# gchq/annchor

Hardware: AMD Instinct MI355X
Metric: knn_graph_builds_per_s (1 / Annchor.fit() wall-clock; BASELINE: k-NN graph build time + recall@k) (higher is better)
Workload: dtype int32 bit-vectors (Levenshtein) + f64 (bounds/regression/selection); 1 GPU; load_strings Levenshtein N=1600 n_anchors=15 k=25 p_work=0.12 niters=2; parallelism=one GPU

## Files before the change

### annchor_amd/csrc/model.hip

```cpp
#include "common.h"

#define OLS_T 256
#define ERR_CAP 8192

int ann_dev_flags(annchor_ctx *c)
{
    ANN_TRY(ann_reserve(c, c->dev_flags, sizeof(int32_t) * 16));
    if (!c->dev_flags_clean) {
        ANN_CHECK_HIP(c, hipMemsetAsync(c->dev_flags.p, 0, sizeof(int32_t) * 16, c->stream));
        c->dev_flags_clean = true;
    }
    return ANNCHOR_OK;
}

__device__ __forceinline__ double block_sum(double v, double *sh )
{
#pragma unroll
    for (int off = 32; off > 0; off >>= 1) v += __shfl_xor(v, off);
    __syncthreads();
    if ((threadIdx.x & 63) == 0) sh[threadIdx.x >> 6] = v;
    __syncthreads();
    double s = sh[0];
    for (int w = 1; w < OLS_T / 64; ++w) s += sh[w];
    return s;
}

#define OLS_RCOND 1e-13
struct ModelEdges { double e[MAXBINS + 1]; };
__global__ __launch_bounds__(OLS_T) void k_ols_bins(const double *__restrict__ sfeat, const double *__restrict__ sy, int64_t m,
                                                   DeviceModel *__restrict__ dm, double *__restrict__ scratch, int64_t cap,
                                                   int32_t *__restrict__ flags, ModelEdges ed, int nb)
{
    __shared__ double sh[OLS_T / 64];
    __shared__ int wcnt[OLS_T / 64];
    __shared__ int base_sh;
    const int b = blockIdx.x, tid = threadIdx.x, lane = tid & 63, wave = tid >> 6;
    const double lo = ed.e[b], hi = ed.e[b + 1];
    if (tid == 0) dm->status[b] = 0;
    if (b == 0) {
        if (tid >= nb && tid < MAXBINS) { dm->status[tid] = 0; dm->rows[tid] = 0; }
        if (tid <= nb) dm->reg.e[tid] = ed.e[tid];
        if (tid == 0) { dm->reg.nb = nb; dm->err_status = 0; }
    }
    double *A = scratch + (size_t)b * 4 * cap;
    double *col[4] = {A, A + cap, A + 2 * cap, A + 3 * cap};
    if (tid == 0) base_sh = 0;
    __syncthreads();
    for (int64_t t0 = 0; t0 < m; t0 += OLS_T) {
        const int64_t t = t0 + tid;
        const double d = t < m ? sfeat[4 * t + 2] : 0.0;
        const bool in = t < m && d > lo && d <= hi;
        const unsigned long long bal = __ballot(in);
        if (lane == 0) wcnt[wave] = __popcll(bal);
        __syncthreads();
        int off = base_sh;
        for (int w = 0; w < wave; ++w) off += wcnt[w];
        if (in) {
            const int r = off + __popcll(bal & ((1ull << lane) - 1ull));
            col[0][r] = sfeat[4 * t]; col[1][r] = sfeat[4 * t + 1]; col[2][r] = d; col[3][r] = sy[t];
        }
        __syncthreads();
        if (tid == 0) base_sh += wcnt[0] + wcnt[1] + wcnt[2] + wcnt[3];
        __syncthreads();
    }
    const int n = base_sh;
    if (tid == 0) dm->rows[b] = n;
    if (n < 3) {
        if (tid == 0) {
            dm->status[b] = 2; dm->reg.w[b][0] = dm->reg.w[b][1] = dm->reg.w[b][2] = 0.0; dm->reg.c[b] = 0.0;
            atomicMax(&flags[1], 2);
        }
        return;
    }
    double mean[4];
    for (int k = 0; k < 4; ++k) {
        double s = 0.0;
        for (int r = tid; r < n; r += OLS_T) s += col[k][r];
        mean[k] = block_sum(s, sh) / (double)n;
    }
    for (int k = 0; k < 4; ++k)
        for (int r = tid; r < n; r += OLS_T) col[k][r] -= mean[k];
    __syncthreads();
    double Rd[3], R01 = 0, R02 = 0, R12 = 0, qy[3];
    double cmax = 0.0;
    for (int j = 0; j < 3; ++j) {
        double s = 0.0;
        for (int r = j + tid; r < n; r += OLS_T) s += col[j][r] * col[j][r];
        const double sigma = block_sum(s, sh);
        const double ajj = col[j][j];
        const double alpha = ajj > 0.0 ? -sqrt(sigma) : sqrt(sigma);
        Rd[j] = alpha;
        cmax = fmax(cmax, fabs(alpha));
        const double vtv = 2.0 * (sigma - alpha * ajj);
        __syncthreads();
        if (tid == 0) col[j][j] = ajj - alpha;
        __syncthreads();
        for (int k = j + 1; k < 4; ++k) {
            double dsum = 0.0;
            for (int r = j + tid; r < n; r += OLS_T) dsum += col[j][r] * col[k][r];
            const double dot = block_sum(dsum, sh);
            const double tau = vtv > 0.0 ? 2.0 * dot / vtv : 0.0;
            for (int r = j + tid; r < n; r += OLS_T) col[k][r] -= tau * col[j][r];
            __syncthreads();
        }
        if (j == 0) { R01 = col[1][0]; R02 = col[2][0]; }
        if (j == 1) R12 = col[2][1];
        qy[j] = col[3][j];
    }
    if (tid == 0) {
        const double tol = 1e-10 * cmax;
        int st = 0;
        for (int j = 0; j < 3; ++j)
            if (!(fabs(Rd[j]) > tol)) st = 1;
        double w2 = 0, w1 = 0, w0 = 0;
        if (!st) {
            w2 = qy[2] / Rd[2];
            w1 = (qy[1] - R12 * w2) / Rd[1];
            w0 = ((qy[0] - R01 * w1) - R02 * w2) / Rd[0];
        } else {
            double M[3][3] = {{Rd[0], R01, R02}, {0.0, Rd[1], R12}, {0.0, 0.0, Rd[2]}};
            double V[3][3] = {{1, 0, 0}, {0, 1, 0}, {0, 0, 1}};
            bool conv = false;
            for (int sweep = 0; sweep < 40 && !conv; ++sweep) {
                conv = true;
                for (int p = 0; p < 2; ++p)
                    for (int q = p + 1; q < 3; ++q) {
                        double al = 0, be = 0, ga = 0;
                        for (int r = 0; r < 3; ++r) { al += M[r][p] * M[r][p]; be += M[r][q] * M[r][q]; ga += M[r][p] * M[r][q]; }
                        if (ga == 0.0 || al <= 1e-40 * be || be <= 1e-40 * al || fabs(ga) <= 4.5e-16 * sqrt(al * be)) continue;
                        conv = false;
                        const double zeta = (be - al) / (2.0 * ga);
                        const double tt = (zeta >= 0.0 ? 1.0 : -1.0) / (fabs(zeta) + sqrt(1.0 + zeta * zeta));
                        const double cs = 1.0 / sqrt(1.0 + tt * tt), sn = cs * tt;
                        for (int r = 0; r < 3; ++r) {
                            const double mp = M[r][p], mq = M[r][q];
                            M[r][p] = cs * mp - sn * mq; M[r][q] = sn * mp + cs * mq;
                            const double vp = V[r][p], vq = V[r][q];
                            V[r][p] = cs * vp - sn * vq; V[r][q] = sn * vp + cs * vq;
                        }
                    }
            }
            double sg2[3], smax2 = 0.0;
            for (int i = 0; i < 3; ++i) {
                sg2[i] = (M[0][i] * M[0][i] + M[1][i] * M[1][i]) + M[2][i] * M[2][i];
                smax2 = fmax(smax2, sg2[i]);
            }
            if (conv && smax2 > 0.0) {
                double w[3] = {0, 0, 0};
                for (int i = 0; i < 3; ++i)
                    if (sg2[i] > (OLS_RCOND * OLS_RCOND) * smax2) {
                        const double coef = ((M[0][i] * qy[0] + M[1][i] * qy[1]) + M[2][i] * qy[2]) / sg2[i];
                        for (int r = 0; r < 3; ++r) w[r] += coef * V[r][i];
                    }
                w0 = w[0]; w1 = w[1]; w2 = w[2];
                st = 0;
            } else if (smax2 == 0.0) st = 0;
        }
        dm->status[b] = st;
        if (st) atomicMax(&flags[1], st);
        dm->reg.w[b][0] = w0; dm->reg.w[b][1] = w1; dm->reg.w[b][2] = w2;
        dm->reg.c[b] = mean[3] - ((mean[0] * w0 + mean[1] * w1) + mean[2] * w2);
    }
}

extern "C" int annchor_fit_regression_device(annchor_ctx *c, const double *bins, int32_t nb, int32_t first_iteration, int32_t is_metric)
{
    if (!c || !bins) return ANNCHOR_EINVAL;
    ANN_REQUIRE(c, c->have_features, ANNCHOR_EINVAL, "features not computed");
    ANN_REQUIRE(c, nb >= 1 && nb <= MAXBINS, ANNCHOR_ELIMIT, "1..%d partitions supported", MAXBINS);
    ANN_REQUIRE(c, first_iteration || c->have_RA, ANNCHOR_EINVAL, "RefineApprox not initialised");
    ANN_REQUIRE(c, c->nsamp > 0 && c->sfeat.p && c->sy.p, ANNCHOR_ESTATE, "no device-resident sample (annchor_sample_pairs_device)");
    ANN_REQUIRE(c, c->sfeat_rows == c->nsamp, ANNCHOR_ESTATE,
                "the current sample of %lld pairs has no device-resident feature rows (%lld rows from an earlier annchor_sample_pairs_device)",
                (long long)c->nsamp, (long long)c->sfeat_rows);
    ANN_CHECK_HIP(c, hipSetDevice(c->device));
    const int64_t m = c->nsamp;
    ANN_TRY(ann_reserve(c, c->model, sizeof(DeviceModel)));
    ANN_TRY(ann_reserve(c, c->ols_scratch, sizeof(double) * 4 * (size_t)m * (size_t)nb));
    ANN_TRY(ann_dev_flags(c));
    DeviceModel *dm = c->model.as<DeviceModel>();
    ModelEdges ed;
    for (int k = 0; k <= MAXBINS; ++k) ed.e[k] = k <= nb ? bins[k] : 0.0;
    static_assert(MAXBINS + 1 <= OLS_T, "one thread per edge");
    {
        ProfScope ps(c, "ols_partitions", (double)m * 40.0 * nb);
        k_ols_bins<<<nb, OLS_T, 0, c->stream>>>(c->sfeat.as<double>(), c->sy.as<double>(), m, dm, c->ols_scratch.as<double>(), m,
                                                c->dev_flags.as<int32_t>(), ed, nb);
    }
    ANN_CHECK_HIP(c, hipGetLastError());
    c->model_fitted = true; c->model_nb = nb; c->errs_on_device = false; c->model_cache_valid = false;
    return ann_predict_merge_device(c, &dm->reg, first_iteration, is_metric);
}

__device__ __forceinline__ unsigned long long err_key(double v) { return ann_key_asc(v); }

__global__ __launch_bounds__(1024) void k_err_sort(const double *__restrict__ sfeat, const double *__restrict__ sy,
                                                   const double *__restrict__ spred, int64_t m, DeviceModel *__restrict__ dm,
                                                   double *__restrict__ errs, int nb, int32_t *__restrict__ flags,
                                                   int64_t *__restrict__ errptr_out)
{
    extern __shared__ unsigned long long keys[];
    __shared__ int wcnt[16];
    __shared__ int base_sh;
    __shared__ int pcnt[MAXBINS];
    const int b = blockIdx.x, tid = threadIdx.x, lane = tid & 63, wave = tid >> 6;
    const double lo = dm->reg.e[b], hi = dm->reg.e[b + 1];
    if (tid < MAXBINS) pcnt[tid] = 0;
    __syncthreads();
    for (int64_t t = tid; t < m; t += 1024) {
        const double d = sfeat[4 * t + 2];
        for (int q = 0; q < nb; ++q)
            if (d >= dm->reg.e[q] && d <= dm->reg.e[q + 1]) atomicAdd(&pcnt[q], 1);
    }
    __syncthreads();
    const int n = pcnt[b];
    if (tid == 0) dm->rows[b] = n;
    int64_t my_at = 0;
    for (int q = 0; q < b; ++q) my_at += pcnt[q];
    if (b == 0 && tid == 0) {
        int64_t at = 0;
        int st = 0;
        for (int q = 0; q < nb; ++q) {
            dm->errptr[q] = at;
            errptr_out[q] = at;
            const int64_t r = pcnt[q];
            if (r == 0) st = max(st, 1);
            if (r > ERR_CAP) st = max(st, 2);
            at += r;
        }
        dm->errptr[nb] = at;
        errptr_out[nb] = at;
        dm->err_status = st;
        if (st) flags[2] = st;
    }
    if (n == 0 || n > ERR_CAP) return;
    int P2 = 1;
    while (P2 < n) P2 <<= 1;
    for (int t = tid; t < P2; t += 1024) keys[t] = ~0ull;
    if (tid == 0) base_sh = 0;
    __syncthreads();
    for (int64_t t0 = 0; t0 < m; t0 += 1024) {
        const int64_t t = t0 + tid;
        const double d = t < m ? sfeat[4 * t + 2] : 0.0;
        const bool in = t < m && d >= lo && d <= hi;
        const unsigned long long bal = __ballot(in);
        if (lane == 0) wcnt[wave] = __popcll(bal);
        __syncthreads();
        int off = base_sh;
        for (int w = 0; w < wave; ++w) off += wcnt[w];
        if (in) keys[off + __popcll(bal & ((1ull << lane) - 1ull))] = err_key(sy[t] - spred[t]);
        __syncthreads();
        if (tid == 0) {
            int s = 0;
            for (int w = 0; w < 16; ++w) s += wcnt[w];
            base_sh += s;
        }
        __syncthreads();
    }
    for (int k = 2; k <= P2; k <<= 1)
        for (int j = k >> 1; j > 0; j >>= 1) {
            for (int t = tid; t < P2; t += 1024) {
                const int p = t ^ j;
                if (p > t) {
                    const unsigned long long a = keys[t], bb = keys[p];
                    const bool up = (t & k) == 0;
                    if ((a > bb) == up) { keys[t] = bb; keys[p] = a; }
                }
            }
            __syncthreads();
        }
    double *out = errs + my_at;
    for (int t = tid; t < n; t += 1024) out[t] = ann_key_asc_inv(keys[t]);
}

extern "C" int annchor_fit_errors_device(annchor_ctx *c)
{
    if (!c) return ANNCHOR_EINVAL;
    ANN_REQUIRE(c, c->model_fitted && c->nsamp > 0 && c->spred.p, ANNCHOR_ESTATE, "annchor_fit_regression_device first");
    ANN_REQUIRE(c, c->sfeat_rows == c->nsamp, ANNCHOR_ESTATE, "the sample changed since annchor_fit_regression_device");
    ANN_CHECK_HIP(c, hipSetDevice(c->device));
    const int nb = c->model_nb;
    const int64_t m = c->nsamp;
    DeviceModel *dm = c->model.as<DeviceModel>();
    ANN_TRY(ann_reserve(c, c->errs, sizeof(double) * 2 * (size_t)m));
    ANN_TRY(ann_reserve(c, c->errptr, sizeof(int64_t) * (size_t)(MAXBINS + 1)));
    {
        ProfScope ps(c, "error_residual_lists", (double)m * 32.0 * nb);
        const size_t lds = sizeof(unsigned long long) * ERR_CAP;
        ANN_CHECK_HIP(c, hipFuncSetAttribute((const void *)k_err_sort, hipFuncAttributeMaxDynamicSharedMemorySize, (int)lds));
        k_err_sort<<<nb, 1024, lds, c->stream>>>(c->sfeat.as<double>(), c->sy.as<double>(), c->spred.as<double>(), m, dm, c->errs.as<double>(),
                                                 nb, c->dev_flags.as<int32_t>(), c->errptr.as<int64_t>());
    }
    ANN_CHECK_HIP(c, hipGetLastError());
    c->errs_on_device = true; c->model_cache_valid = false;
    return ANNCHOR_OK;
}

extern "C" int annchor_model_download(annchor_ctx *c, double *W, double *cc, int32_t *status, int64_t *err_ptr, int32_t *flags)
{
    if (!c || !W || !cc || !status || !flags) return ANNCHOR_EINVAL;
    ANN_REQUIRE(c, c->model.p && c->model_nb > 0, ANNCHOR_ESTATE, "no model on this context");
    ANN_CHECK_HIP(c, hipSetDevice(c->device));
    DeviceModel h;
    int32_t f[16];
    ANN_TRY(ann_dev_flags(c));
    ANN_TRY(ann_d2h2(c, &h, c->model.p, sizeof h, f, c->dev_flags.p, sizeof f));
    for (int b = 0; b < c->model_nb; ++b) {
        W[3 * b] = h.reg.w[b][0]; W[3 * b + 1] = h.reg.w[b][1]; W[3 * b + 2] = h.reg.w[b][2];
        cc[b] = h.reg.c[b];
        status[b] = h.status[b];
    }
    if (err_ptr)
        for (int b = 0; b <= c->model_nb; ++b) err_ptr[b] = h.errptr[b];
    flags[0] = f[0]; flags[1] = f[1]; flags[2] = f[2];
    if (f[0] | f[1] | f[2]) {
        ANN_CHECK_HIP(c, hipMemsetAsync(c->dev_flags.p, 0, sizeof(int32_t) * 16, c->stream));
    }
    return ANNCHOR_OK;
}

int ann_model_prefetch_begin(annchor_ctx *c, unsigned char *at, size_t room, size_t *used)
{
    *used = 0;
    c->model_cache_valid = false;
    if (!(c->model_fitted && c->errs_on_device && c->model.p && c->errs.p && c->model_nb > 0)) return ANNCHOR_OK;
    const size_t eb = sizeof(double) * 2 * (size_t)c->nsamp;
    const size_t off_f = (sizeof(DeviceModel) + 63) & ~(size_t)63, off_e = off_f + 64;
    if (off_e + eb > room) return ANNCHOR_OK;
    ANN_TRY(ann_dev_flags(c));
    ANN_CHECK_HIP(c, hipMemcpyAsync(at, c->model.p, sizeof(DeviceModel), hipMemcpyDeviceToHost, c->stream));
    ANN_CHECK_HIP(c, hipMemcpyAsync(at + off_f, c->dev_flags.p, sizeof(int32_t) * 16, hipMemcpyDeviceToHost, c->stream));
    if (eb) ANN_CHECK_HIP(c, hipMemcpyAsync(at + off_e, c->errs.p, eb, hipMemcpyDeviceToHost, c->stream));
    c->model_cache_errs = eb;
    *used = off_e + eb;
    return ANNCHOR_OK;
}
void ann_model_prefetch_end(annchor_ctx *c, const unsigned char *at, size_t used)
{
    if (!used) return;
    c->model_cache.assign(at, at + used);
    c->model_cache_valid = true;
}

extern "C" int annchor_model_download_with_errors(annchor_ctx *c, double *W, double *cc, int32_t *status, int64_t *err_ptr, int32_t *flags,
                                                  double *errs, int64_t errs_cap, int64_t *n_errs)
{
    if (!c || !W || !cc || !status || !flags || !err_ptr || !errs || !n_errs) return ANNCHOR_EINVAL;
    ANN_REQUIRE(c, c->model.p && c->model_nb > 0, ANNCHOR_ESTATE, "no model on this context");
    ANN_REQUIRE(c, c->errs_on_device && c->errs.p, ANNCHOR_ESTATE, "no device-resident residual lists");
    ANN_CHECK_HIP(c, hipSetDevice(c->device));
    size_t eb = sizeof(double) * (size_t)std::min<int64_t>(errs_cap, 2 * c->nsamp);
    const size_t off_f = (sizeof(DeviceModel) + 63) & ~(size_t)63, off_e = off_f + 64;
    const bool cached = c->model_cache_valid && c->model_cache.size() >= off_e + c->model_cache_errs;
    c->model_cache_valid = false;
    if (!cached && (!c->pin || off_e + eb > annchor_ctx::PIN_DL_BYTES)) {
        ANN_TRY(annchor_model_download(c, W, cc, status, err_ptr, flags));
        *n_errs = err_ptr[c->model_nb];
        ANN_REQUIRE(c, *n_errs <= errs_cap, ANNCHOR_EINVAL, "residual lists hold %lld entries, room for %lld", (long long)*n_errs, (long long)errs_cap);
        return annchor_errors_download(c, errs, *n_errs);
    }
    ANN_TRY(ann_dev_flags(c));
    const unsigned char *slot = c->pin + (size_t)annchor_ctx::PIN_SLOTS * annchor_ctx::PIN_SLOT_BYTES;
    if (cached) {
        slot = c->model_cache.data();
        eb = c->model_cache_errs;
    } else {
        unsigned char *dst = c->pin + (size_t)annchor_ctx::PIN_SLOTS * annchor_ctx::PIN_SLOT_BYTES;
        ANN_CHECK_HIP(c, hipMemcpyAsync(dst, c->model.p, sizeof(DeviceModel), hipMemcpyDeviceToHost, c->stream));
        ANN_CHECK_HIP(c, hipMemcpyAsync(dst + off_f, c->dev_flags.p, sizeof(int32_t) * 16, hipMemcpyDeviceToHost, c->stream));
        if (eb) ANN_CHECK_HIP(c, hipMemcpyAsync(dst + off_e, c->errs.p, eb, hipMemcpyDeviceToHost, c->stream));
        ANN_CHECK_HIP(c, ann_sync(c, __func__));
    }
    const DeviceModel &h = *reinterpret_cast<const DeviceModel *>(slot);
    const int32_t *f = reinterpret_cast<const int32_t *>(slot + off_f);
    for (int b = 0; b < c->model_nb; ++b) {
        W[3 * b] = h.reg.w[b][0]; W[3 * b + 1] = h.reg.w[b][1]; W[3 * b + 2] = h.reg.w[b][2];
        cc[b] = h.reg.c[b];
        status[b] = h.status[b];
    }
    for (int b = 0; b <= c->model_nb; ++b) err_ptr[b] = h.errptr[b];
    flags[0] = f[0]; flags[1] = f[1]; flags[2] = f[2];
    *n_errs = err_ptr[c->model_nb];
    if (*n_errs < 0 || (size_t)*n_errs * sizeof(double) > eb || *n_errs > errs_cap) *n_errs = -1;
    else memcpy(errs, slot + off_e, sizeof(double) * (size_t)*n_errs);
    if (f[0] | f[1] | f[2]) ANN_CHECK_HIP(c, hipMemsetAsync(c->dev_flags.p, 0, sizeof(int32_t) * 16, c->stream));
    return ANNCHOR_OK;
}

extern "C" int annchor_errors_download(annchor_ctx *c, double *errs, int64_t n_errs)
{
    if (!c || (n_errs > 0 && !errs)) return ANNCHOR_EINVAL;
    ANN_REQUIRE(c, c->errs_on_device && c->errs.p, ANNCHOR_ESTATE, "no device-resident residual lists");
    if (n_errs == 0) return ANNCHOR_OK;
    ANN_CHECK_HIP(c, hipSetDevice(c->device));
    return ann_d2h(c, errs, c->errs.p, sizeof(double) * (size_t)n_errs);
}
```

Before: 369.1 graphs/s.

## Restructure OLS and error-sort kernels with LDS staging, fused reductions, register bitonic sort

```diff
diff --git a/annchor_amd/csrc/model.hip b/annchor_amd/csrc/model.hip
--- a/annchor_amd/csrc/model.hip
+++ b/annchor_amd/csrc/model.hip
@@ -1,7 +1,14 @@
 #include "common.h"
+#include <atomic>
 
 #define OLS_T 256
+#define OLS_PER 8
+#define OLS_TRIP (OLS_T * OLS_PER)
+#define OLS_LDS_ROWS 4096
 #define ERR_CAP 8192
+#define ERR_T 1024
+#define ERR_PER 8
+#define ERR_TRIP (ERR_T * ERR_PER)
 
 int ann_dev_flags(annchor_ctx *c)
 {
@@ -13,27 +20,108 @@
     return ANNCHOR_OK;
 }
 
-__device__ __forceinline__ double block_sum(double v, double *sh )
-{
-#pragma unroll
-    for (int off = 32; off > 0; off >>= 1) v += __shfl_xor(v, off);
+static int ann_lds_once(annchor_ctx *c, const void *fn, int which, size_t bytes)
+{
+    static std::atomic<bool> done[2][64];
+    const int d = c->device;
+    const bool memo = d >= 0 && d < 64;
+    if (memo && done[which][d].load(std::memory_order_acquire)) return ANNCHOR_OK;
+    ANN_CHECK_HIP(c, hipFuncSetAttribute(fn, hipFuncAttributeMaxDynamicSharedMemorySize, (int)bytes));
+    if (memo) done[which][d].store(true, std::memory_order_release);
+    return ANNCHOR_OK;
+}
+
+template <int NV> __device__ __forceinline__ void block_sums(double (&v)[NV], double (*sh)[4][OLS_T / 64], int &par)
+{
+#pragma unroll
+    for (int k = 0; k < NV; ++k) {
+#pragma unroll
+        for (int off = 32; off > 0; off >>= 1) v[k] += __shfl_xor(v[k], off);
+    }
+    if ((threadIdx.x & 63) == 0) {
+#pragma unroll
+        for (int k = 0; k < NV; ++k) sh[par][k][threadIdx.x >> 6] = v[k];
+    }
     __syncthreads();
-    if ((threadIdx.x & 63) == 0) sh[threadIdx.x >> 6] = v;
-    __syncthreads();
-    double s = sh[0];
-    for (int w = 1; w < OLS_T / 64; ++w) s += sh[w];
-    return s;
+#pragma unroll
+    for (int k = 0; k < NV; ++k) {
+        double s = sh[par][k][0];
+#pragma unroll
+        for (int w = 1; w < OLS_T / 64; ++w) s += sh[par][k][w];
+        v[k] = s;
+    }
+    par ^= 1;
 }
 
 #define OLS_RCOND 1e-13
 struct ModelEdges { double e[MAXBINS + 1]; };
+struct OlsFactor { double mean[4], Rd[3], R01, R02, R12, qy[3], cmax; };
+
+__device__ __forceinline__ void ols_factor(double *A, const size_t cap, const int n, double (*sh)[4][OLS_T / 64], int &par, OlsFactor &f)
+{
+    const int tid = threadIdx.x;
+    double *col[4] = {A, A + cap, A + 2 * cap, A + 3 * cap};
+    double s4[4] = {0.0, 0.0, 0.0, 0.0};
+    for (int r = tid; r < n; r += OLS_T) {
+#pragma unroll
+        for (int k = 0; k < 4; ++k) s4[k] += col[k][r];
+    }
+    block_sums<4>(s4, sh, par);
+#pragma unroll
+    for (int k = 0; k < 4; ++k) f.mean[k] = s4[k] / (double)n;
+    double sg[1] = {0.0};
+    for (int r = tid; r < n; r += OLS_T) {
+        const double x0 = col[0][r] - f.mean[0];
+        col[0][r] = x0;
+        sg[0] += x0 * x0;
+#pragma unroll
+        for (int k = 1; k < 4; ++k) col[k][r] -= f.mean[k];
+    }
+    f.R01 = f.R02 = f.R12 = 0.0;
+    f.cmax = 0.0;
+#pragma unroll
+    for (int j = 0; j < 3; ++j) {
+        if (j > 0) {
+            sg[0] = 0.0;
+            for (int r = j + tid; r < n; r += OLS_T) sg[0] += col[j][r] * col[j][r];
+        }
+        block_sums<1>(sg, sh, par);
+        const double sigma = sg[0];
+        const double ajj = col[j][j];
+        const double alpha = ajj > 0.0 ? -sqrt(sigma) : sqrt(sigma);
+        f.Rd[j] = alpha;
+        f.cmax = fmax(f.cmax, fabs(alpha));
+        const double vtv = 2.0 * (sigma - alpha * ajj);
+        const double v0 = ajj - alpha;
+        double dot[3] = {0.0, 0.0, 0.0};
+        for (int r = j + tid; r < n; r += OLS_T) {
+            const double vj = r == j ? v0 : col[j][r];
+#pragma unroll
+            for (int k = j + 1; k < 4; ++k) dot[k - 1] += vj * col[k][r];
+        }
+        block_sums<3>(dot, sh, par);
+        double tau[3];
+#pragma unroll
+        for (int k = j + 1; k < 4; ++k) tau[k - 1] = vtv > 0.0 ? 2.0 * dot[k - 1] / vtv : 0.0;
+        for (int r = j + tid; r < n; r += OLS_T) {
+            const double vj = r == j ? v0 : col[j][r];
+#pragma unroll
+            for (int k = j + 1; k < 4; ++k) col[k][r] -= tau[k - 1] * vj;
+        }
+        __syncthreads();
+        if (j == 0) { f.R01 = col[1][0]; f.R02 = col[2][0]; }
+        if (j == 1) f.R12 = col[2][1];
+        f.qy[j] = col[3][j];
+    }
+}
+
 __global__ __launch_bounds__(OLS_T) void k_ols_bins(const double *__restrict__ sfeat, const double *__restrict__ sy, int64_t m,
                                                    DeviceModel *__restrict__ dm, double *__restrict__ scratch, int64_t cap,
-                                                   int32_t *__restrict__ flags, ModelEdges ed, int nb)
-{
-    __shared__ double sh[OLS_T / 64];
-    __shared__ int wcnt[OLS_T / 64];
-    __shared__ int base_sh;
+                                                   int32_t *__restrict__ flags, ModelEdges ed, int nb, int lrows)
+{
+    extern __shared__ double ols_lds[];
+    __shared__ double sh[2][4][OLS_T / 64];
+    __shared__ int wcnt[2][OLS_PER][OLS_T / 64];
     const int b = blockIdx.x, tid = threadIdx.x, lane = tid & 63, wave = tid >> 6;
     const double lo = ed.e[b], hi = ed.e[b + 1];
     if (tid == 0) dm->status[b] = 0;
@@ -42,28 +130,48 @@
         if (tid <= nb) dm->reg.e[tid] = ed.e[tid];
         if (tid == 0) { dm->reg.nb = nb; dm->err_status = 0; }
     }
-    double *A = scratch + (size_t)b * 4 * cap;
-    double *col[4] = {A, A + cap, A + 2 * cap, A + 3 * cap};
-    if (tid == 0) base_sh = 0;
-    __syncthreads();
-    for (int64_t t0 = 0; t0 < m; t0 += OLS_T) {
-        const int64_t t = t0 + tid;
-        const double d = t < m ? sfeat[4 * t + 2] : 0.0;
-        const bool in = t < m && d > lo && d <= hi;
-        const unsigned long long bal = __ballot(in);
-        if (lane == 0) wcnt[wave] = __popcll(bal);
+    double *G = scratch + (size_t)b * 4 * cap;
+    const double2 *__restrict__ sf2 = reinterpret_cast<const double2 *>(sfeat);
+    const unsigned long long below = (1ull << lane) - 1ull;
+    int base = 0, wp = 0;
+    for (int64_t t0 = 0; t0 < m; t0 += OLS_TRIP) {
+        double2 fa[OLS_PER], fb[OLS_PER];
+        double yv[OLS_PER];
+        unsigned long long bal[OLS_PER];
+#pragma unroll
+        for (int i = 0; i < OLS_PER; ++i) {
+            const int64_t t = t0 + i * OLS_T + tid, tc = t < m ? t : m - 1;
+            fa[i] = sf2[2 * tc]; fb[i] = sf2[2 * tc + 1]; yv[i] = sy[tc];
+        }
+#pragma unroll
+        for (int i = 0; i < OLS_PER; ++i) {
+            const int64_t t = t0 + i * OLS_T + tid;
+            bal[i] = __ballot(t < m && fb[i].x > lo && fb[i].x <= hi);
+            if (lane == 0) wcnt[wp][i][wave] = __popcll(bal[i]);
+        }
         __syncthreads();
-        int off = base_sh;
-        for (int w = 0; w < wave; ++w) off += wcnt[w];
-        if (in) {
-            const int r = off + __popcll(bal & ((1ull << lane) - 1ull));
-            col[0][r] = sfeat[4 * t]; col[1][r] = sfeat[4 * t + 1]; col[2][r] = d; col[3][r] = sy[t];
-        }
-        __syncthreads();
-        if (tid == 0) base_sh += wcnt[0] + wcnt[1] + wcnt[2] + wcnt[3];
-        __syncthreads();
-    }
-    const int n = base_sh;
+        int run = base;
+#pragma unroll
+        for (int i = 0; i < OLS_PER; ++i) {
+            int off = 0;
+#pragma unroll
+            for (int w = 0; w < OLS_T / 64; ++w) {
+                if (w == wave) off = run;
+                run += wcnt[wp][i][w];
+            }
+            if ((bal[i] >> lane) & 1ull) {
+                const int r = off + __popcll(bal[i] & below);
+                if (r < lrows) {
+                    ols_lds[r] = fa[i].x; ols_lds[lrows + r] = fa[i].y; ols_lds[2 * lrows + r] = fb[i].x; ols_lds[3 * lrows + r] = yv[i];
+                } else {
+                    G[r] = fa[i].x; G[cap + r] = fa[i].y; G[2 * cap + r] = fb[i].x; G[3 * cap + r] = yv[i];
+                }
+            }
+        }
+        base = run;
+        wp ^= 1;
+    }
+    const int n = base;
     if (tid == 0) dm->rows[b] = n;
     if (n < 3) {
         if (tid == 0) {
@@ -72,41 +180,20 @@
         }
         return;
     }
-    double mean[4];
-    for (int k = 0; k < 4; ++k) {
-        double s = 0.0;
-        for (int r = tid; r < n; r += OLS_T) s += col[k][r];
-        mean[k] = block_sum(s, sh) / (double)n;
-    }
-    for (int k = 0; k < 4; ++k)
-        for (int r = tid; r < n; r += OLS_T) col[k][r] -= mean[k];
     __syncthreads();
-    double Rd[3], R01 = 0, R02 = 0, R12 = 0, qy[3];
-    double cmax = 0.0;
-    for (int j = 0; j < 3; ++j) {
-        double s = 0.0;
-        for (int r = j + tid; r < n; r += OLS_T) s += col[j][r] * col[j][r];
-        const double sigma = block_sum(s, sh);
-        const double ajj = col[j][j];
-        const double alpha = ajj > 0.0 ? -sqrt(sigma) : sqrt(sigma);
-        Rd[j] = alpha;
-        cmax = fmax(cmax, fabs(alpha));
-        const double vtv = 2.0 * (sigma - alpha * ajj);
+    OlsFactor f;
+    int par = 0;
+    if (n <= lrows) ols_factor(ols_lds, (size_t)lrows, n, sh, par, f);
+    else {
+        for (int r = tid; r < lrows; r += OLS_T) {
+#pragma unroll
+            for (int k = 0; k < 4; ++k) G[(size_t)k * cap + r] = ols_lds[k * lrows + r];
+        }
         __syncthreads();
-        if (tid == 0) col[j][j] = ajj - alpha;
-        __syncthreads();
-        for (int k = j + 1; k < 4; ++k) {
-            double dsum = 0.0;
-            for (int r = j + tid; r < n; r += OLS_T) dsum += col[j][r] * col[k][r];
-            const double dot = block_sum(dsum, sh);
-            const double tau = vtv > 0.0 ? 2.0 * dot / vtv : 0.0;
-            for (int r = j + tid; r < n; r += OLS_T) col[k][r] -= tau * col[j][r];
-            __syncthreads();
-        }
-        if (j == 0) { R01 = col[1][0]; R02 = col[2][0]; }
-        if (j == 1) R12 = col[2][1];
-        qy[j] = col[3][j];
-    }
+        ols_factor(G, (size_t)cap, n, sh, par, f);
+    }
+    const double *mean = f.mean, *Rd = f.Rd, *qy = f.qy;
+    const double R01 = f.R01, R02 = f.R02, R12 = f.R12, cmax = f.cmax;
     if (tid == 0) {
         const double tol = 1e-10 * cmax;
         int st = 0;
@@ -182,10 +269,13 @@
     ModelEdges ed;
     for (int k = 0; k <= MAXBINS; ++k) ed.e[k] = k <= nb ? bins[k] : 0.0;
     static_assert(MAXBINS + 1 <= OLS_T, "one thread per edge");
+    const int lrows = (int)std::min<int64_t>(m, OLS_LDS_ROWS);
+    ANN_TRY(ann_lds_once(c, (const void *)k_ols_bins, 0, sizeof(double) * 4 * OLS_LDS_ROWS));
     {
         ProfScope ps(c, "ols_partitions", (double)m * 40.0 * nb);
-        k_ols_bins<<<nb, OLS_T, 0, c->stream>>>(c->sfeat.as<double>(), c->sy.as<double>(), m, dm, c->ols_scratch.as<double>(), m,
-                                                c->dev_flags.as<int32_t>(), ed, nb);
+        k_ols_bins<<<nb, OLS_T, sizeof(double) * 4 * (size_t)lrows, c->stream>>>(c->sfeat.as<double>(), c->sy.as<double>(), m, dm,
+                                                                              c->ols_scratch.as<double>(), m, c->dev_flags.as<int32_t>(),
+                                                                              ed, nb, lrows);
     }
     ANN_CHECK_HIP(c, hipGetLastError());
     c->model_fitted = true; c->model_nb = nb; c->errs_on_device = false; c->model_cache_valid = false;
@@ -194,23 +284,119 @@
 
 __device__ __forceinline__ unsigned long long err_key(double v) { return ann_key_asc(v); }
 
-__global__ __launch_bounds__(1024) void k_err_sort(const double *__restrict__ sfeat, const double *__restrict__ sy,
-                                                   const double *__restrict__ spred, int64_t m, DeviceModel *__restrict__ dm,
-                                                   double *__restrict__ errs, int nb, int32_t *__restrict__ flags,
-                                                   int64_t *__restrict__ errptr_out)
+template <int E> __device__ __forceinline__ void err_sort_store(unsigned long long *buf, const int n, const int P2, double *__restrict__ out)
+{
+    const int tid = threadIdx.x;
+    unsigned long long r[E];
+#pragma unroll
+    for (int s = 0; s < E; ++s) r[s] = s * ERR_T + tid < n ? buf[s * ERR_T + tid] : ~0ull;
+    int p = 1;
+    for (int k = 2; k <= P2; k <<= 1) {
+#pragma unroll
+        for (int js = E / 2; js >= 1; js >>= 1) {
+            if (js * ERR_T < k) {
+#pragma unroll
+                for (int s = 0; s < E; ++s)
+                    if ((s & js) == 0) {
+                        const bool up = ((s * ERR_T + tid) & k) == 0;
+                        const unsigned long long a = r[s], bb = r[s | js];
+                        if ((a > bb) == up) { r[s] = bb; r[s | js] = a; }
+                    }
+            }
+        }
+        for (int j = min(k >> 1, ERR_T / 2); j >= 64; j >>= 1) {
+            unsigned long long *w = buf + p * ERR_CAP;
+#pragma unroll
+            for (int s = 0; s < E; ++s) w[s * ERR_T + tid] = r[s];
+            __syncthreads();
+#pragma unroll
+            for (int s = 0; s < E; ++s) {
+                const int e = s * ERR_T + tid;
+                const unsigned long long o = w[e ^ j];
+                const bool take_min = ((e & j) == 0) == ((e & k) == 0);
+                r[s] = take_min ? (o < r[s] ? o : r[s]) : (o > r[s] ? o : r[s]);
+            }
+            p ^= 1;
+        }
+        for (int j = min(k >> 1, 32); j >= 1; j >>= 1) {
+#pragma unroll
+            for (int s = 0; s < E; ++s) {
+                const int e = s * ERR_T + tid;
+                const unsigned long long o = __shfl_xor(r[s], j);
+                const bool take_min = ((e & j) == 0) == ((e & k) == 0);
+                r[s] = take_min ? (o < r[s] ? o : r[s]) : (o > r[s] ? o : r[s]);
+            }
+        }
+    }
+#pragma unroll
+    for (int s = 0; s < E; ++s)
+        if (s * ERR_T + tid < n) out[s * ERR_T + tid] = ann_key_asc_inv(r[s]);
+}
+
+__global__ __launch_bounds__(ERR_T) void k_err_sort(const double *__restrict__ sfeat, const double *__restrict__ sy,
+                                                    const double *__restrict__ spred, int64_t m, DeviceModel *__restrict__ dm,
+                                                    double *__restrict__ errs, int nb, int32_t *__restrict__ flags,
+                                                    int64_t *__restrict__ errptr_out)
 {
     extern __shared__ unsigned long long keys[];
-    __shared__ int wcnt[16];
-    __shared__ int base_sh;
+    __shared__ int wtot[2][ERR_T / 64];
+    __shared__ int pcw[ERR_T / 64][MAXBINS];
     __shared__ int pcnt[MAXBINS];
     const int b = blockIdx.x, tid = threadIdx.x, lane = tid & 63, wave = tid >> 6;
+    const double elo = dm->reg.e[lane < nb ? lane : 0], ehi = dm->reg.e[lane < nb ? lane + 1 : 0];
     const double lo = dm->reg.e[b], hi = dm->reg.e[b + 1];
-    if (tid < MAXBINS) pcnt[tid] = 0;
+    const unsigned long long below = (1ull << lane) - 1ull;
+    int mycnt = 0, base = 0, wp = 0;
+    for (int64_t t0 = 0; t0 < m; t0 += ERR_TRIP) {
+        double d[ERR_PER], res[ERR_PER];
+        unsigned long long bal[ERR_PER];
+#pragma unroll
+        for (int i = 0; i < ERR_PER; ++i) {
+            const int64_t t = t0 + i * ERR_T + tid, tc = t < m ? t : m - 1;
+            d[i] = sfeat[4 * tc + 2];
+            res[i] = sy[tc] - spred[tc];
+            if (t >= m) d[i] = __longlong_as_double(-1ll);
+        }
+        int wsum = 0;
+#pragma unroll
+        for (int i = 0; i < ERR_PER; ++i) {
+            bal[i] = __ballot(d[i] >= lo && d[i] <= hi);
+            wsum += __popcll(bal[i]);
+        }
+        if (lane == 0) wtot[wp][wave] = wsum;
+        for (int q = 0; q < nb; ++q) {
+            const double ql = __shfl(elo, q), qh = __shfl(ehi, q);
+            int cq = 0;
+#pragma unroll
+            for (int i = 0; i < ERR_PER; ++i) cq += __popcll(__ballot(d[i] >= ql && d[i] <= qh));
+            if (lane == q) mycnt += cq;
+        }
+        __syncthreads();
+        int off = base, tot = 0;
+#pragma unroll
+        for (int w = 0; w < ERR_T / 64; ++w) {
+            const int x = wtot[wp][w];
+            if (w < wave) off += x;
+            tot += x;
+        }
+#pragma unroll
+        for (int i = 0; i < ERR_PER; ++i) {
+            if ((bal[i] >> lane) & 1ull) {
+                const int at = off + __popcll(bal[i] & below);
+                if (at < ERR_CAP) keys[at] = err_key(res[i]);
+            }
+            off += __popcll(bal[i]);
+        }
+        base += tot;
+        wp ^= 1;
+    }
+    pcw[wave][lane] = mycnt;
     __syncthreads();
-    for (int64_t t = tid; t < m; t += 1024) {
-        const double d = sfeat[4 * t + 2];
-        for (int q = 0; q < nb; ++q)
-            if (d >= dm->reg.e[q] && d <= dm->reg.e[q + 1]) atomicAdd(&pcnt[q], 1);
+    if (tid < MAXBINS) {
+        int s = 0;
+#pragma unroll
+        for (int w = 0; w < ERR_T / 64; ++w) s += pcw[w][tid];
+        pcnt[tid] = s;
     }
     __syncthreads();
     const int n = pcnt[b];
@@ -236,41 +422,11 @@
     if (n == 0 || n > ERR_CAP) return;
     int P2 = 1;
     while (P2 < n) P2 <<= 1;
-    for (int t = tid; t < P2; t += 1024) keys[t] = ~0ull;
-    if (tid == 0) base_sh = 0;
-    __syncthreads();
-    for (int64_t t0 = 0; t0 < m; t0 += 1024) {
-        const int64_t t = t0 + tid;
-        const double d = t < m ? sfeat[4 * t + 2] : 0.0;
-        const bool in = t < m && d >= lo && d <= hi;
-        const unsigned long long bal = __ballot(in);
-        if (lane == 0) wcnt[wave] = __popcll(bal);
-        __syncthreads();
-        int off = base_sh;
-        for (int w = 0; w < wave; ++w) off += wcnt[w];
-        if (in) keys[off + __popcll(bal & ((1ull << lane) - 1ull))] = err_key(sy[t] - spred[t]);
-        __syncthreads();
-        if (tid == 0) {
-            int s = 0;
-            for (int w = 0; w < 16; ++w) s += wcnt[w];
-            base_sh += s;
-        }
-        __syncthreads();
-    }
-    for (int k = 2; k <= P2; k <<= 1)
-        for (int j = k >> 1; j > 0; j >>= 1) {
-            for (int t = tid; t < P2; t += 1024) {
-                const int p = t ^ j;
-                if (p > t) {
-                    const unsigned long long a = keys[t], bb = keys[p];
-                    const bool up = (t & k) == 0;
-                    if ((a > bb) == up) { keys[t] = bb; keys[p] = a; }
-                }
-            }
-            __syncthreads();
-        }
     double *out = errs + my_at;
-    for (int t = tid; t < n; t += 1024) out[t] = ann_key_asc_inv(keys[t]);
+    if (P2 <= ERR_T) err_sort_store<1>(keys, n, P2, out);
+    else if (P2 == 2 * ERR_T) err_sort_store<2>(keys, n, P2, out);
+    else if (P2 == 4 * ERR_T) err_sort_store<4>(keys, n, P2, out);
+    else err_sort_store<8>(keys, n, P2, out);
 }
 
 extern "C" int annchor_fit_errors_device(annchor_ctx *c)
@@ -284,12 +440,12 @@
     DeviceModel *dm = c->model.as<DeviceModel>();
     ANN_TRY(ann_reserve(c, c->errs, sizeof(double) * 2 * (size_t)m));
     ANN_TRY(ann_reserve(c, c->errptr, sizeof(int64_t) * (size_t)(MAXBINS + 1)));
+    const size_t lds = sizeof(unsigned long long) * 2 * ERR_CAP;
+    ANN_TRY(ann_lds_once(c, (const void *)k_err_sort, 1, lds));
     {
         ProfScope ps(c, "error_residual_lists", (double)m * 32.0 * nb);
-        const size_t lds = sizeof(unsigned long long) * ERR_CAP;
-        ANN_CHECK_HIP(c, hipFuncSetAttribute((const void *)k_err_sort, hipFuncAttributeMaxDynamicSharedMemorySize, (int)lds));
-        k_err_sort<<<nb, 1024, lds, c->stream>>>(c->sfeat.as<double>(), c->sy.as<double>(), c->spred.as<double>(), m, dm, c->errs.as<double>(),
-                                                 nb, c->dev_flags.as<int32_t>(), c->errptr.as<int64_t>());
+        k_err_sort<<<nb, ERR_T, lds, c->stream>>>(c->sfeat.as<double>(), c->sy.as<double>(), c->spred.as<double>(), m, dm, c->errs.as<double>(),
+                                                  nb, c->dev_flags.as<int32_t>(), c->errptr.as<int64_t>());
     }
     ANN_CHECK_HIP(c, hipGetLastError());
     c->errs_on_device = true; c->model_cache_valid = false;
```

Result: faster. 378.2 graphs/s, median of 6 (+2.4%).
